# VeeraKarthick609/ImageCaptioner

Hardware: NVIDIA B200
Metric: kd_train_samples_per_sec (higher is better)
Workload: dtype bf16

## Files before the change

### imagecaptioner_b200/_ops.py

```python
from __future__ import annotations

import ctypes
import os
from typing import List, Optional, Sequence

import torch

_HERE = os.path.dirname(os.path.abspath(__file__))
LIB_PATH = os.environ.get("B2C_LIB") or os.path.join(_HERE, "lib", "libb2c.so")

B2C_MAX_LAYERS = 4
B2C_F32, B2C_BF16 = 0, 1
B2C_WS_TRAIN, B2C_WS_DECODE, B2C_WS_ATTN, B2C_WS_REFINE, B2C_WS_PROJ = 0, 1, 2, 3, 4
ABI_VERSION = 5
B2C_BWD_DEFER_JOIN = 1

c_f32p = ctypes.c_void_p


class B2CShape(ctypes.Structure):
    _fields_ = [(n, ctypes.c_int32) for n in ("B", "T", "S", "E", "H", "L", "V")]


_PARAM_FIELDS = (
    [("embedding", c_f32p), ("attn_w", c_f32p), ("attn_b", c_f32p), ("comb_w", c_f32p), ("comb_b", c_f32p)]
    + [(n, c_f32p * B2C_MAX_LAYERS) for n in ("w_ih", "w_hh", "b_ih", "b_hh")]
    + [("out0_w", c_f32p), ("out0_b", c_f32p), ("out3_w", c_f32p), ("out3_b", c_f32p)]
)


# ... 148 lines not shown
    return st


def _master(params: Sequence[torch.Tensor]) -> List[torch.Tensor]:
    out = []
    for p in params:
        q = p.detach()
        if q.dtype != torch.float32 or not q.is_contiguous():
            q = q.float().contiguous()
        out.append(q)
    return out


class CallOptions:

    def __init__(self, grad_dest=None, defer_join=False, after_backward=None, seed_dev=None, background_ctas=0):
        self.grad_dest, self.defer_join, self.after_backward, self.seed_dev = grad_dest, defer_join, after_backward, seed_dev
        self.background_ctas = background_ctas
        self.join_pending = False


_NO_OPTIONS = CallOptions()


def _options(opts) -> CallOptions:
    return opts if opts is not None else _NO_OPTIONS


def _dropout(p, seed, opts) -> B2CDropout:
    sd = opts.seed_dev
    return B2CDropout(float(p), int(seed), sd.data_ptr() if (sd is not None and float(p) > 0) else None)

# ... 120 lines not shown
        ctx.mark_non_differentiable(attw)
        return logits, hid, attw

    @staticmethod
    def backward(ctx, dlogits, dhid, _dattw):
        lib = load_library()
        shape, code, drop, L, ws, f, cap, master, hid, attw, feats_dtype, pdtypes, opts = ctx.b2c
        cdt = f.dtype
        if dlogits is None:
            dlogits = torch.zeros(shape.T, shape.B, shape.V, dtype=cdt, device=f.device)
        dlogits = dlogits.to(cdt).contiguous()
        if dhid is not None:
            dhid = dhid.to(cdt).contiguous()
        grads, all_direct = _grad_buffers(ctx.b2c_params, master, opts)
        defer = opts.defer_join and all_direct and all(dt == torch.float32 for dt in pdtypes)
        dfeats = torch.empty(shape.B, shape.S, shape.E, dtype=torch.float32, device=f.device)
        prm = _fill_struct(B2CParams(), master, L)
        grd = _fill_struct(B2CGrads(), grads, L)
        _check(lib.b2c_decoder_backward(ctypes.byref(shape), ctypes.byref(prm), f.data_ptr(), cap.data_ptr(), hid.data_ptr(), attw.data_ptr(),
                                        dlogits.data_ptr(), _ptr(dhid), ctypes.byref(grd), dfeats.data_ptr(), ws.data_ptr(), ws.numel(),
                                        code, ctypes.byref(drop), B2C_BWD_DEFER_JOIN if defer else 0, _stream()),
               "b2c_decoder_backward")
        if defer:
            opts.join_pending = True
        if opts.after_backward is not None:
            opts.after_backward()
        grads = [g if g.dtype == dt else g.to(dt) for g, dt in zip(grads, pdtypes)]
        dfe = dfeats if feats_dtype == torch.float32 else dfeats.to(feats_dtype)
        return (dfe, None, None, None, None, None, None, None, None, *grads)


def greedy_decode(feats: torch.Tensor, params: Sequence[torch.Tensor], L: int, max_len: int, start_id: int, end_id: int,
                  compute_dtype: torch.dtype = torch.float32):
    lib = load_library()
    _require_cuda(feats, "image_features")
    B, S, E = feats.shape
# ... 339 lines not shown
```

### imagecaptioner_b200/csrc/api.cu

```cuda
#include <stdlib.h>
#include "gemm.cuh"
#include "loss_kernels.cuh"
#include "decoder_kernels.cuh"
#include "recurrent.cuh"
#include "recur_cluster.cuh"
#include "refine_kernels.cuh"
#include "mha_mma.cuh"
#include "optim_kernels.cuh"

using namespace b2c;

namespace {

constexpr int MAXL = B2C_MAX_LAYERS;
constexpr int COLSUM_RS = 160;

int check_device() {
  static int cached = 1;
  if (cached <= 0) return cached;
  int dev = 0;
  B2C_CUDA(cudaGetDevice(&dev));
  int major = 0;
  B2C_CUDA(cudaDeviceGetAttribute(&major, cudaDevAttrComputeCapabilityMajor, dev));
  if (major != 10) { cached = B2C_EARCH; return set_err(B2C_EARCH, "b2c kernels are built for sm_100a only; device has compute capability major %d", major); }
// ... 25 lines not shown
template <typename T> struct Weights {
  T *Wf, *Wh, *Wce, *Wcc, *W1, *W2, *Wih0, *We; T* Wcat[MAXL]; float* bcat[MAXL]; float* bx;
  T* Wuh;
  void carve(Carver& c, const B2CShape& s) {
    Wf = c.take<T>((size_t)s.E * s.E); Wh = c.take<T>((size_t)s.E * s.H);
    Wce = c.take<T>((size_t)s.E * s.E); Wcc = c.take<T>((size_t)s.E * s.E);
    W1 = c.take<T>((size_t)s.E * s.H); W2 = c.take<T>((size_t)s.V * s.E);
    Wih0 = c.take<T>((size_t)4 * s.H * s.E); We = c.take<T>((size_t)4 * s.H * s.E); bx = c.take<float>((size_t)4 * s.H);
    for (int k = 0; k < s.L; ++k) { Wcat[k] = c.take<T>((size_t)4 * s.H * (in_dim(s, k) + s.H)); bcat[k] = c.take<float>((size_t)4 * s.H); }
    Wuh = c.take<T>((size_t)(s.E + 4 * s.H) * s.H);
  }
};

template <typename T, typename TC>
int gemm(cudaStream_t st, int M, int N, int K, const T* A, long lda, int a_mn, const T* B, long ldb, int b_mn,
         TC* C, long ldc, float beta = 0.f, const float* bias = nullptr, int relu = 0, float alpha = 1.f, int row_unperm_h = 0);

template <typename T>
int pack_params(const B2CShape& s, const B2CParams& p, const Weights<T>& w, cudaStream_t st) {
  B2C_CHECK_ARG(p.embedding && p.attn_w && p.attn_b && p.comb_w && p.comb_b && p.out0_w && p.out0_b && p.out3_w && p.out3_b, "NULL parameter pointer");
  PackTable tab; tab.n = 0;
  auto add = [&](const float* src, void* dst, int rows, int cols, long lds, long ldd, int perm_h = 0, const float* src2 = nullptr, int as_float = 0) {
    PackSeg& g = tab.seg[tab.n++]; g.src = src; g.dst = dst; g.src2 = src2; g.rows = rows; g.cols = cols; g.lds = lds; g.ldd = ldd; g.as_float = as_float; g.perm_h = perm_h;
  };
  const int E = s.E, H = s.H;
  add(p.attn_w, w.Wh, E, H, H + E, H);
  add(p.attn_w + H, w.Wf, E, E, H + E, E);
  add(p.comb_w, w.Wce, E, E, 2 * E, E);
  add(p.comb_w + E, w.Wcc, E, E, 2 * E, E);
  add(p.out0_w, w.W1, E, H, H, H);
  add(p.out3_w, w.W2, s.V, E, E, E);
// ... 96 lines not shown
  void carve(void* base, const B2CShape& s) {
    Carver c{reinterpret_cast<unsigned char*>(base), 0};
    const size_t B = s.B, S = s.S, E = s.E, H = s.H;
    w.carve(c, s);
    P = c.take<float>(B * S * E); emb = c.take<T>(B * E); u = c.take<float>(B * E); G0 = c.take<T>(B * 4 * H); o1 = c.take<T>(B * E);
    for (int k = 0; k < s.L; ++k) { xh[k] = c.take<T>(2 * B * (in_dim(s, k) + H)); this->c[k] = c.take<float>(B * H); }
    logits = c.take<float>(B * (size_t)s.V); cur = c.take<int64_t>(B); done = c.take<int32_t>(B);
    amax_v = c.take<float>(B * (size_t)cdiv(s.V, 32)); amax_i = c.take<int>(B * (size_t)cdiv(s.V, 32));
    bytes = align_up(c.off, 256);
  }
};


template <typename T, typename TC>
int gemm(cudaStream_t st, int M, int N, int K, const T* A, long lda, int a_mn, const T* B, long ldb, int b_mn,
         TC* C, long ldc, float beta, const float* bias, int relu, float alpha, int row_unperm_h) {
  GemmArgs g{M, N, K, alpha, beta, A, lda, a_mn, B, ldb, b_mn, C, ldc, bias, relu};
  g.row_unperm_h = row_unperm_h;
  return Gemm<T, TC>::run(g, st);
}
template <typename T>
int gemm_lstm(cudaStream_t st, int M, int H, int K, const T* A, long lda, const T* Wcat, long ldb, const LstmEpi& le) {
  GemmArgs g{M, 4 * H, K, 1.f, 0.f, A, lda, 0, Wcat, ldb, 0, nullptr, 4 * H, nullptr, 0};
  g.lstm = &le;
  return Gemm<T, float>::run(g, st);
}

inline int ew_grid(long n) { long g = (n + 255) / 256; if (g > 148 * 8) g = 148 * 8; if (g < 1) g = 1; return (int)g; }

template <typename T>
int colsum(cudaStream_t st, const T* A, long rows, int cols, long ld, float* partial, float* out, float* out2 = nullptr, int unperm_h = 0) {
  if (ld == cols && cols % 8 == 0 && ((uintptr_t)A & 15) == 0 && rows >= 256) {
    const int gx = cdiv(cols, 256);
// ... 294 lines not shown
  return 0;
}



inline int bg_ctas() { static int v = -1; if (v < 0) { const char* e = getenv("B2C_BG_CTAS"); v = e ? atoi(e) : 10; } return v; }
inline bool attn_post_occ3() { static int v = -1; if (v < 0) { const char* e = getenv("B2C_POST_OCC3"); v = (e && e[0] == '0') ? 0 : 1; } return v != 0; }
inline int wgrad_chunks() { static int v = -1; if (v < 0) { const char* e = getenv("B2C_WGRAD_CHUNKS"); v = e ? atoi(e) : 0; } return v; }

template <typename T>
int decoder_backward_impl(const B2CShape& s, const B2CParams& p, const T* feats, const int64_t* cap, const T* hid_top,
                          const float* attw, const T* dlogits, const T* dhid, const B2CGrads& g, float* dfeats,
                          void* ws, size_t ws_bytes, const B2CDropout& dr, cudaStream_t st, int flags) {
  TrainWs<T> W; W.carve(ws, s);
  B2C_CHECK_ARG(ws_bytes >= W.bytes, "workspace too small: %zu < %zu", ws_bytes, W.bytes);
  B2C_CHECK_ARG(g.embedding && g.attn_w && g.attn_b && g.comb_w && g.comb_b && g.out0_w && g.out0_b && g.out3_w && g.out3_b && dfeats, "NULL gradient pointer");
  const int B = s.B, Tn = s.T, S = s.S, E = s.E, H = s.H, L = s.L, V = s.V;
  const long TB = (long)Tn * B;
  const float inv_keep = dr.p > 0.f ? 1.0f / (1.0f - dr.p) : 1.0f;
  SubStreams* hs = nullptr;
  B2C_TRY(get_substreams(&hs));
  cudaStream_t side = hs->s[MAX_SUB - 1];
  for (int k = 0; k < L; ++k) B2C_CHECK_ARG(g.w_ih[k] && g.w_hh[k] && g.b_ih[k] && g.b_hh[k], "NULL LSTM gradient pointer (layer %d)", k);
  B2C_CUDA(cudaEventRecord(hs->ev[3], st));
  B2C_CUDA(cudaStreamWaitEvent(side, hs->ev[3], 0));
  B2C_CUDA(cudaMemsetAsync(W.dxh0, 0, (size_t)TB * (E + H) * sizeof(float), side));
  for (int k = 1; k < L; ++k) B2C_CUDA(cudaMemsetAsync(W.dxh[k], 0, (size_t)TB * 2 * H * sizeof(float), side));
  B2C_CUDA(cudaEventRecord(hs->ev[3], side));
  B2C_TRY((gemm<T, T>(st, (int)TB, E, V, dlogits, V, 0, W.w.W2, E, 1, W.do1, E)));
  relu_bwd_inplace_kernel<T><<<ew_grid(TB * E), 256, 0, st>>>(W.do1, W.o1, TB * E, inv_keep);
  B2C_LAUNCH_CHECK("relu_bwd_inplace_kernel");
  B2C_CUDA(cudaEventRecord(hs->fork, st));
  B2C_CUDA(cudaStreamWaitEvent(side, hs->fork, 0));
  {
    GemmCapScope bg(bg_ctas());
    B2C_TRY((gemm<T, float>(side, V, E, (int)TB, dlogits, V, 1, W.o1, E, 1, g.out3_w, E)));
    B2C_TRY(colsum<T>(side, dlogits, TB, V, V, W.partial_side, g.out3_b));
    B2C_TRY((gemm<T, float>(side, E, H, (int)TB, W.do1, E, 1, hid_top, H, 1, g.out0_w, H)));
    B2C_TRY(colsum<T>(side, W.do1, TB, E, E, W.partial_side, g.out0_b));
  }
  B2C_CUDA(cudaEventRecord(hs->join[MAX_SUB - 1], side));
  B2C_TRY((gemm<T, float>(st, (int)TB, H, E, W.do1, E, 0, W.w.W1, H, 1, W.dHext, H)));
  B2C_CUDA(cudaStreamWaitEvent(st, hs->ev[3], 0));
  SubPlan sp;
  B2C_TRY(fork_subs(sp, B, st));
  auto weight_grads = [&](cudaStream_t s2, long r0, long r1, float beta) -> int {
    const int K = (int)(r1 - r0);
    for (int k = 1; k < L; ++k) {
      const int in = in_dim(s, k), ld = in + H;
      B2C_TRY((gemm<T, float>(s2, 4 * H, in, K, W.dgates[k] + r0 * 4 * H, 4 * H, 1, W.xh[k] + r0 * ld, ld, 1, g.w_ih[k], in, beta, nullptr, 0, 1.f, H)));
      B2C_TRY((gemm<T, float>(s2, 4 * H, H, K, W.dgates[k] + r0 * 4 * H, 4 * H, 1, W.xh[k] + r0 * ld + in, ld, 1, g.w_hh[k], H, beta, nullptr, 0, 1.f, H)));
    }
    B2C_TRY((gemm<T, float>(s2, 4 * H, E, K, W.dgates[0] + r0 * 4 * H, 4 * H, 1, W.xh[0] + r0 * (E + H), E + H, 1, W.dWx32, E, beta)));
    B2C_TRY((gemm<T, float>(s2, 4 * H, E, K, W.dgates[0] + r0 * 4 * H, 4 * H, 1, W.emb + r0 * E, E, 1, W.dWe32, E, beta)));
    B2C_TRY((gemm<T, float>(s2, 4 * H, H, K, W.dgates[0] + r0 * 4 * H, 4 * H, 1, W.xh[0] + r0 * (E + H) + E, E + H, 1, g.w_hh[0], H, beta, nullptr, 0, 1.f, H)));
    return 0;
  };
  const int n_chunks = (sp.ns == 1 && bg_ctas() > 0) ? wgrad_chunks() : 0;
  const int chunk_steps = n_chunks > 0 ? cdiv(Tn, n_chunks) : 0;
  long wg_done_from = TB;
  bool wg_any = false;
  pdl_full_dependency_next();
  for (int t = Tn - 1; t >= 0; --t) {
    const bool last = (t == Tn - 1);
    for (int i = 0; i < sp.ns; ++i) {
      cudaStream_t ss = sp.st[i];
      const long b0 = sp.b0[i];
      const int Bh = sp.bn[i];
      const long row = (long)t * B + b0;
      for (int k = L - 1; k >= 0; --k) {
// ... 11 lines not shown
      }
      const float* dctx_t = W.dxh0 + row * (E + H);
      T* du_t = W.du + row * E;
      B2C_TRY(attn_bwd<T>(ss, Bh, S, E, W.P + b0 * S * E, feats + b0 * S * E, W.u + row * E, attw + row * S, dctx_t, (long)(E + H), W.ds + row * S, du_t));
      if (t > 0) B2C_TRY((gemm<T, T>(ss, Bh, H, E, du_t, E, 0, W.w.Wh, H, 1, W.dq + b0 * H, H)));
    }
    if (chunk_steps > 0 && t > 0 && (Tn - t) % chunk_steps == 0 && t >= chunk_steps) {
      B2C_CUDA(cudaEventRecord(hs->ev[0], st));
      B2C_CUDA(cudaStreamWaitEvent(side, hs->ev[0], 0));
      GemmCapScope bg(bg_ctas());
      B2C_TRY(weight_grads(side, (long)t * B, wg_done_from, wg_any ? 1.f : 0.f));
      wg_done_from = (long)t * B; wg_any = true;
    }
  }
  B2C_TRY(join_subs(sp));
  B2C_CUDA(cudaEventRecord(hs->ev[1], st));
  B2C_CUDA(cudaStreamWaitEvent(side, hs->ev[1], 0));
  B2C_TRY(weight_grads(side, 0, wg_done_from, wg_any ? 1.f : 0.f));
  for (int k = 0; k < L; ++k) B2C_TRY(colsum<T>(side, W.dgates[k], TB, 4 * H, 4 * H, W.partial_side, g.b_ih[k], g.b_hh[k], H));
  {
    cast_f32_kernel<T><<<ew_grid((long)4 * H * E / 8), 256, 0, side>>>(W.dWx32, W.dWxT, (long)4 * H * E);
    B2C_LAUNCH_CHECK("cast_f32_kernel");
    cast_f32_kernel<T><<<ew_grid((long)4 * H * E / 8), 256, 0, side>>>(W.dWe32, W.dWeT, (long)4 * H * E);
    B2C_LAUNCH_CHECK("cast_f32_kernel");
    B2C_TRY((gemm<T, float>(side, 4 * H, E, E, W.dWxT, E, 0, W.w.Wcc, E, 0, g.w_ih[0], E, 0.f, nullptr, 0, 1.f, H)));
    B2C_TRY((gemm<T, float>(side, 4 * H, E, E, W.dWeT, E, 0, W.w.Wce, E, 0, g.w_ih[0], E, 1.f, nullptr, 0, 1.f, H)));
    rank1_add_kernel<<<ew_grid((long)4 * H * E), 256, 0, side>>>(g.w_ih[0], g.b_ih[0], p.comb_b, (long)4 * H, E);
    B2C_LAUNCH_CHECK("rank1_add_kernel");
    B2C_TRY((gemm<T, float>(side, E, E, 4 * H, W.w.Wih0, E, 1, W.dWeT, E, 1, g.comb_w, 2 * E)));
    B2C_TRY((gemm<T, float>(side, E, E, 4 * H, W.w.Wih0, E, 1, W.dWxT, E, 1, g.comb_w + E, 2 * E)));
    B2C_CUDA(cudaMemsetAsync(g.comb_b, 0, (size_t)E * sizeof(float), side));
    bias_fold_bwd_kernel<<<dim3(cdiv(E, 32), 32), 256, 0, side>>>(p.w_ih[0], g.b_ih[0], 4 * H, E, g.comb_b);
    B2C_LAUNCH_CHECK("bias_fold_bwd_kernel");
    B2C_TRY((gemm<T, float>(side, (int)TB, E, 4 * H, W.dgates[0], 4 * H, 0, W.w.We, E, 1, W.demb, E)));
    B2C_CUDA(cudaMemsetAsync(g.embedding, 0, (size_t)V * E * sizeof(float), side));
    embedding_scatter_add_kernel<<<ew_grid(TB * E), 256, 0, side>>>(W.demb, cap, TB, E, V, g.embedding);
    B2C_LAUNCH_CHECK("embedding_scatter_add_kernel");
  }
  const int inL = in_dim(s, L - 1), ldL = inL + H;
  B2C_TRY((gemm<T, float>(side, E, H, (int)TB, W.du, E, 1, W.xh[L - 1] + inL, ldL, 1, g.attn_w, H + E)));
  if (Tn <= 24) {
    const int splits = 1, per = cdiv(S, splits), TP = (Tn + 3) & ~3;
    const size_t psmem = (size_t)2 * per * TP * 4;
    if (Tn <= 20 && attn_post_occ3()) {
      B2C_TRY(set_smem(attn_post_reg_kernel<T, 20>, psmem));
      attn_post_reg_kernel<T, 20><<<dim3(B, splits), ATT_THREADS, psmem, st>>>(W.P, W.u, W.dxh0, (long)(E + H), attw, W.ds, Tn, B, S, E, W.dP, dfeats);
    } else {
      B2C_TRY(set_smem(attn_post_reg_kernel<T, 24>, psmem));
      attn_post_reg_kernel<T, 24><<<dim3(B, splits), ATT_THREADS, psmem, st>>>(W.P, W.u, W.dxh0, (long)(E + H), attw, W.ds, Tn, B, S, E, W.dP, dfeats);
    }
    B2C_LAUNCH_CHECK("attn_post_reg_kernel");
  } else {
    const size_t smem = (size_t)Tn * (2 * E + 2 * S) * 4;
    B2C_TRY(set_smem(attn_post_kernel<T>, smem));
    attn_post_kernel<T><<<B, ATT_THREADS, smem, st>>>(W.P, W.u, W.dxh0, (long)(E + H), attw, W.ds, Tn, B, S, E, W.dP, dfeats);
    B2C_LAUNCH_CHECK("attn_post_kernel");
  }
  B2C_CUDA(cudaEventRecord(hs->ev[2], st));
  B2C_TRY((gemm<T, float>(st, B * S, E, E, W.dP, E, 0, W.w.Wf, E, 1, dfeats, E, 1.f)));
  B2C_CUDA(cudaStreamWaitEvent(side, hs->ev[2], 0));
  B2C_TRY((gemm<T, float>(side, E, E, B * S, W.dP, E, 1, feats, E, 1, g.attn_w + H, H + E)));
  B2C_TRY(colsum<T>(side, W.dP, (long)B * S, E, E, W.partial_side, g.attn_b));
  B2C_CUDA(cudaEventRecord(hs->join[MAX_SUB - 1], side));
  if (flags & B2C_BWD_DEFER_JOIN) return 0;
  B2C_CUDA(cudaStreamWaitEvent(st, hs->join[MAX_SUB - 1], 0));
  return 0;
}


inline bool fuse_argmax_off() { static const bool off = getenv("B2C_DECODE_LOGITS") != nullptr; return off; }

template <typename T>
int greedy_decode_impl(const B2CShape& s, const B2CParams& p, const T* feats, int64_t start_id, int64_t end_id,
                       int64_t* tokens, int32_t* lengths, void* ws, size_t ws_bytes, cudaStream_t st) {
  DecodeWs<T> W; W.carve(ws, s);
  B2C_CHECK_ARG(ws_bytes >= W.bytes, "workspace too small: %zu < %zu", ws_bytes, W.bytes);
  const int B = s.B, Tn = s.T, S = s.S, E = s.E, H = s.H, L = s.L, V = s.V;
// ... 710 lines not shown
```

### imagecaptioner_b200/csrc/gemm.cuh

```cuda
#pragma once
#include "common.cuh"

namespace b2c {

struct LstmEpi {
  int enabled, H;
  const void* addend;
  const float* bias;
  const float* c_prev; float* c_out;
  void* gates_out;
  void* h_rec; long ld_rec; void* h_next; long ld_next; void* h_top; long ld_top;
  float drop_p; unsigned long long seed; unsigned int site; long row_base;
  const unsigned long long* seed_dev;
  const float* addend32; long ld_addend32;
};

constexpr int EVAL_PART_FLOATS = 8;
struct EvalEpi { const float* teacher; const int64_t* targets; float* parts; float inv_temp; int nparts; int cols_per_part; };

struct ArgmaxEpi { float* pmax; int* pidx; int nparts; int cols_per_part; };
inline LstmEpi pack_argmax(const ArgmaxEpi& a) {
  LstmEpi le{};
  le.enabled = 2; le.H = a.nparts; le.c_out = a.pmax; le.gates_out = a.pidx; le.ld_rec = a.cols_per_part;
  return le;
// ... 515 lines not shown
          }
#pragma unroll
          for (int j = 0; j < 32; ++j) if (colb + j < N && v[j] > best) { best = v[j]; bidx = colb + j; }
        }
      }
      if (grow < M) {
        const int part = (n0 + half * C_PER * CH) / (C_PER * CH);
        if (part < nparts) { pmax[(long)grow * nparts + part] = best; pidx[(long)grow * nparts + part] = bidx; }
      }
      tc_fence_before();
      __syncwarp();
      if (lane == 0) mbar_arrive(&tempty_bar[as]);
      continue;
    }
    if constexpr (EPI == 0 || EPI == 4) {
    if (EPI == 4 || ((split ? sizeof(TC) == 4 : beta == 0.f) && vec_ok && m0 + TC_BM <= M && n0 + BN <= N && (((uintptr_t)bias) & 15) == 0)) {
#pragma unroll 1
      for (int ci = half * C_PER; ci < (half + 1) * C_PER && ci < NCHUNK; ++ci) {
        const int c0 = ci * CH;
#pragma unroll
        for (int h = 0; h < CH / 32; ++h) {
          float v[32];
          tmem_ld32(tacc + (uint32_t)(c0 + h * 32), v);
          if (add_bias) {
            const float4* b4 = reinterpret_cast<const float4*>(bias + n0 + c0 + h * 32);
#pragma unroll
            for (int j = 0; j < 8; ++j) {
              const float4 bb = __ldg(b4 + j);
              v[4 * j] = fmaf(alpha, v[4 * j], bb.x); v[4 * j + 1] = fmaf(alpha, v[4 * j + 1], bb.y);
              v[4 * j + 2] = fmaf(alpha, v[4 * j + 2], bb.z); v[4 * j + 3] = fmaf(alpha, v[4 * j + 3], bb.w);
            }
// ... 11 lines not shown
            for (int j = 0; j < 32; j += 8)
              *reinterpret_cast<uint4*>(dst + j * 2) = make_uint4(pack_bf16(v[j], v[j + 1]), pack_bf16(v[j + 2], v[j + 3]), pack_bf16(v[j + 4], v[j + 5]), pack_bf16(v[j + 6], v[j + 7]));
          } else {
#pragma unroll
            for (int j = 0; j < 32; j += 4)
              *reinterpret_cast<uint4*>(dst + j * 4) = make_uint4(__float_as_uint(v[j]), __float_as_uint(v[j + 1]), __float_as_uint(v[j + 2]), __float_as_uint(v[j + 3]));
          }
        }
        __syncwarp();
#pragma unroll
        for (int it = 0; it < 8; ++it) {
          const int r = it * 4 + (lane >> 3), grow = m0 + q * 32 + r;
          const long orow = row_unperm_h ? (long)(grow & 3) * row_unperm_h + (grow >> 2) : (long)grow;
          TC* cp = C + orow * ldc + n0 + c0 + (lane & 7) * PER;
          const uint4 acc = *reinterpret_cast<const uint4*>(my + r * TC_EPI_PITCH + (lane & 7) * 16);
          if (split) {
            asm volatile("red.global.add.v4.f32 [%0], {%1, %2, %3, %4};" :: "l"(cp), "f"(__uint_as_float(acc.x)), "f"(__uint_as_float(acc.y)),
                         "f"(__uint_as_float(acc.z)), "f"(__uint_as_float(acc.w)) : "memory");
          } else {
            *reinterpret_cast<uint4*>(cp) = acc;
          }
        }
        __syncwarp();
      }
      tc_fence_before();
      __syncwarp();
      if (lane == 0) mbar_arrive(&tempty_bar[as]);
      continue;
    }
    if constexpr (EPI == 0) {
#pragma unroll 1
// ... 108 lines not shown
  if (r != CUDA_SUCCESS) return set_err(B2C_ECUDA, "cuTensorMapEncodeTiled failed (%d): ptr=%p inner=%ld outer=%ld ld=%ld box=%d", (int)r, ptr, inner, outer, ld, box_outer);
  return 0;
}

struct GemmArgs {
  int M, N, K;
  float alpha, beta;
  const void* A; long lda; int a_mn;
  const void* B; long ldb; int b_mn;
  void* C; long ldc;
  const float* bias; int relu;
  int row_unperm_h = 0;
  const LstmEpi* lstm = nullptr;
  ArgmaxEpi* amax = nullptr;
  EvalEpi* eval = nullptr;
};

inline bool tc_eligible(const GemmArgs& g) {
  return ((uintptr_t)g.A % 16 == 0) && ((uintptr_t)g.B % 16 == 0) && (g.lda % 8 == 0) && (g.ldb % 8 == 0);
}

struct TcPlan { int bn, splits, kb_per_split; };
inline TcPlan plan_tc(const GemmArgs& g, int elem_c, int sms) {
  const int num_kb = cdiv(g.K, TC_BK);
  const bool can_split = (elem_c == 4) && !g.relu && (g.beta == 0.f || g.beta == 1.f) && (g.lstm == nullptr) && (g.amax == nullptr) && (g.eval == nullptr);
  TcPlan best{64, 1, num_kb}; double best_cost = 1e30;
  const int cand[3] = {256, 128, 64};
  for (int ci = 0; ci < 3; ++ci) {
    const int bn = cand[ci];
    if (bn > 64 && g.N <= bn / 2) continue;
// ... 23 lines not shown
  int saved;
  explicit GemmCapScope(int cap) : saved(gemm_cta_cap()) { gemm_cta_cap() = cap; }
  ~GemmCapScope() { gemm_cta_cap() = saved; }
};
inline int gemm_sms() { const int n = sm_count(), c = gemm_cta_cap(); return (c > 0 && c < n) ? c : n; }

template <int BN, bool A_MN, bool B_MN, typename TC>
int launch_tc(const GemmArgs& g, const TcPlan& plan, cudaStream_t st) {
  CUtensorMap ta, tb;
  if (!A_MN) B2C_TRY(make_tmap_bf16(&ta, g.A, g.K, g.M, g.lda, TC_BM)); else B2C_TRY(make_tmap_bf16(&ta, g.A, g.M, g.K, g.lda, 64));
  if (!B_MN) B2C_TRY(make_tmap_bf16(&tb, g.B, g.K, g.N, g.ldb, BN)); else B2C_TRY(make_tmap_bf16(&tb, g.B, g.N, g.K, g.ldb, 64));
  constexpr bool CAN_LSTM = !A_MN && !B_MN && sizeof(TC) == 4;
  void (*kern)(const CUtensorMap, const CUtensorMap, int, int, int, float, float, TC*, long, const float*, int, int, int, int, int, int, const LstmEpi) =
      gemm_tc_kernel<BN, A_MN, B_MN, TC, 0>;
  int flavour = g.lstm ? ((g.lstm->drop_p > 0.f && g.lstm->h_next) ? 1 : 5) : (g.amax ? 2 : (g.eval ? 3 : 0));
  if (flavour == 0 && fast_only_enabled() && g.M % TC_BM == 0 && g.N % BN == 0 && (plan.splits > 1 ? sizeof(TC) == 4 : g.beta == 0.f) &&
      ((uintptr_t)g.C) % 16 == 0 && (g.ldc * (long)sizeof(TC)) % 16 == 0 && (((uintptr_t)g.bias) & 15) == 0) {
    flavour = 4;
    kern = gemm_tc_kernel<BN, A_MN, B_MN, TC, 4>;
  }
  if (flavour != 0 && flavour != 4) {
    if constexpr (CAN_LSTM) {
      kern = flavour == 1 ? gemm_tc_kernel<BN, A_MN, B_MN, TC, 1> : (flavour == 5 ? gemm_tc_kernel<BN, A_MN, B_MN, TC, 5> :
             (flavour == 2 ? gemm_tc_kernel<BN, A_MN, B_MN, TC, 2> : gemm_tc_kernel<BN, A_MN, B_MN, TC, 3>));
    } else return set_err(B2C_EINVAL, "the fused LSTM / argmax / validation epilogues need K-major operands and the fp32 instantiation");
  }
  static bool attr_set[6] = {false, false, false, false, false, false};
  if (!attr_set[flavour]) {
    B2C_CUDA(cudaFuncSetAttribute(kern, cudaFuncAttributeMaxDynamicSharedMemorySize, (int)TcCfg<BN>::SMEM_BYTES));
    attr_set[flavour] = true;
  }
  const int kb_per_split = plan.kb_per_split, splits = plan.splits;
  if (splits > 1 && g.beta == 0.f)
    B2C_CUDA(cudaMemset2DAsync(g.C, (size_t)g.ldc * sizeof(TC), 0, (size_t)g.N * sizeof(TC), (size_t)g.M, st));
  const int tiles_m = cdiv(g.M, TC_BM), tiles_n = cdiv(g.N, BN);
  const long total = (long)tiles_m * tiles_n * splits;
  const int grid = (int)(total < gemm_sms() ? total : gemm_sms());
  LstmEpi epi = g.lstm ? *g.lstm : LstmEpi{};
  if (g.amax) {
    B2C_CHECK_ARG(!g.lstm && splits == 1 && g.amax->pmax && g.amax->pidx, "argmax epilogue: no K split, no LSTM epilogue, partial buffers required");
    constexpr int CHc = 128 / (int)sizeof(TC), CPER = (BN / CHc + 1) / 2;
    g.amax->cols_per_part = CPER * CHc;
    g.amax->nparts = cdiv(g.N, g.amax->cols_per_part);
    epi = pack_argmax(*g.amax);
  }
  if (g.eval) {
    B2C_CHECK_ARG(!g.lstm && !g.amax && splits == 1 && g.eval->teacher && g.eval->targets && g.eval->parts, "validation epilogue: no K split, no other epilogue, buffers required");
    constexpr int CHc = 128 / (int)sizeof(TC), CPER = (BN / CHc + 1) / 2;
// ... 48 lines not shown
```

### imagecaptioner_b200/graph.py

```python
from __future__ import annotations

import os
from typing import Dict, Optional

import torch

from . import _ops
from .ddp import FlatGradAllReducer


class GraphedKDStep:
    INPUT_KEYS = ("encoder_features", "captions_input", "targets", "teacher_logits", "teacher_features", "teacher_hiddens")

    def __init__(self, model, projector, loss_module, optimizer, reducer: Optional[FlatGradAllReducer], example: Dict[str, torch.Tensor],
                 max_grad_norm: float = 1.0, autocast_dtype: Optional[torch.dtype] = torch.bfloat16, use_graph: bool = True,
                 warmup_steps: int = 3, direct_grads: bool = True):
        self.model, self.projector, self.loss_module = model, projector, loss_module
        self._native_opt = hasattr(optimizer, "flat_param") and hasattr(optimizer, "reducer")
        if self._native_opt:
            if reducer is None:
                reducer = optimizer.reducer
            if reducer is not optimizer.reducer:
                raise ValueError("a FlatAdamW optimizer brings its own gradient buffer: pass reducer=None or optimizer.reducer")
        self.optimizer, self.reducer = optimizer, reducer
# ... 5 lines not shown
        self.static = {k: example[k].clone() for k in self.INPUT_KEYS if example.get(k) is not None}
        self.static["encoder_features"].requires_grad_(True)
        self.out5 = None
        self.graph = None
        self.graph_opt = None
        self.world = reducer.world_size
        self._side = torch.cuda.Stream()
        self._aux = torch.cuda.Stream()
        self._aux_used = False
        self._overlap = False
        self._capturing = False
        self.high_priority_chain = os.environ.get("B2C_CHAIN_PRIORITY", "1") != "0"
        self.defer_weight_grad_join = os.environ.get("B2C_DEFER_JOIN", "1") != "0"
        self.background_ctas = int(os.environ.get("B2C_BG_CTAS", "10"))
        self.direct_grads = direct_grads
        loss_module.assume_unit_grad = True
        dev = self.static["targets"].device
        self.step_counter = torch.zeros(1, dtype=torch.int64, device=dev)
        self._opts = _ops.CallOptions(grad_dest=reducer.grad_views() if direct_grads else None, seed_dev=self.step_counter)
        self._fake_dp = self.world == 1 and os.environ.get("B2C_FAKE_DP", "0") == "1"
        self._multi = self.world > 1 or self._fake_dp
        self.nval = torch.zeros(1, dtype=torch.int32, device=self.static["targets"].device) if self._multi else None
        self._nval_single = torch.zeros(1, dtype=torch.int32, device=self.static["targets"].device) if not self._multi else None
        self.overlap_comm = use_graph and self._multi and os.environ.get("B2C_OVERLAP_COMM", "1") != "0"
        self._early = self._early_segment() if self.overlap_comm else None
        if self.overlap_comm:
            self._comm = torch.cuda.Stream()
            self._ev_count = torch.cuda.Event(external=True)
            self._ev_dec = torch.cuda.Event(external=True)
        if use_graph:
# ... 20 lines not shown
            self._all_reduce(self.nval)
            self.loss_module.n_valid_global = self.nval

    def _modules(self):
        mods = [self.model.decoder, self.projector]
        if getattr(self.model, "use_attention_refinement", False):
            mods.append(self.model.attention_refinement)
        return mods

    def _attach_options(self):
        o = self._opts
        early = self._capturing and self.overlap_comm and self._early is not None
        o.defer_join = self.defer_weight_grad_join and self.direct_grads and (not self._multi or early)
        o.after_backward = self._after_decoder_backward if early else None
        o.background_ctas = self.background_ctas if self._overlap else 0
        for m in self._modules():
            m.b2c_options = o

    def _after_decoder_backward(self):
        main = torch.cuda.current_stream()
        if self._opts.join_pending:
            self._opts.join_pending = False
            self._aux.wait_stream(main)
            with torch.cuda.stream(self._aux):
                _ops.join_side_work()
                self._ev_dec.record()
            self._aux_used = True
        else:
            self._ev_dec.record()

# ... 14 lines not shown
        if feats.grad is not None:
            feats.grad = None
        self._attach_options()
        if self._dropout_active():
            _ops.bump_counter(self.step_counter)
        ctx = torch.autocast("cuda", dtype=self.autocast_dtype) if self.autocast_dtype is not None else torch.autocast("cuda", enabled=False)
        if self._overlap:
            main = torch.cuda.current_stream()
            self._side.wait_stream(main)
            if self._nval_single is not None:
                with torch.cuda.stream(self._side):
                    _ops.count_valid(inp["targets"], self.loss_module.vocab_size or 2 ** 31 - 1, out=self._nval_single)
                self.loss_module.n_valid_global = self._nval_single
            with torch.cuda.stream(self._side), ctx:
                tproj = self.projector(inp["teacher_features"])
            with ctx:
                outputs, enc, hids, _ = self.model(feats, inp["captions_input"])
            main.wait_stream(self._side)
        else:
            with ctx:
                outputs, enc, hids, _ = self.model(feats, inp["captions_input"])
                tproj = self.projector(inp["teacher_features"])
        if self._capturing and self.overlap_comm:
            torch.cuda.current_stream().wait_event(self._ev_count)
        loss, out5 = self.loss_module.forward_device(
            {"logits": outputs, "encoder_features": enc, "hidden_states": hids},
            {"logits": inp["teacher_logits"], "encoder_features": tproj, "hidden_states": inp.get("teacher_hiddens")},
            inp["targets"])
        if self.direct_grads:
            self.reducer.detach_grads()
# ... 117 lines not shown
```

### include/b2c.h

```cpp
#ifndef B2C_H_
#define B2C_H_

#include <stddef.h>
#include <stdint.h>

#ifdef __cplusplus
extern "C" {
#endif

#define B2C_ABI_VERSION 5
#define B2C_MAX_LAYERS 4

enum { B2C_OK = 0, B2C_EINVAL = -1, B2C_EARCH = -2, B2C_ECUDA = -3, B2C_ENOMEM = -4 };
enum { B2C_F32 = 0, B2C_BF16 = 1 };
enum { B2C_WS_TRAIN = 0, B2C_WS_DECODE = 1, B2C_WS_ATTN = 2, B2C_WS_REFINE = 3, B2C_WS_PROJ = 4 };

typedef struct B2CShape { int32_t B, T, S, E, H, L, V; } B2CShape;

typedef struct B2CParams {
  const float* embedding;
  const float* attn_w;  const float* attn_b;
  const float* comb_w;  const float* comb_b;
  const float* w_ih[B2C_MAX_LAYERS]; const float* w_hh[B2C_MAX_LAYERS];
  const float* b_ih[B2C_MAX_LAYERS]; const float* b_hh[B2C_MAX_LAYERS];
// ... 32 lines not shown
int b2c_decoder_prepare(const B2CShape* shape, const B2CParams* params, const int64_t* captions, void* workspace, size_t ws_bytes,
                        int dtype, void* stream);
int b2c_decoder_forward_prepared(const B2CShape* shape, const B2CParams* params, const void* feats, const int64_t* captions,
                        void* logits, void* hidden_top, float* attn_w, void* workspace, size_t ws_bytes,
                        int dtype, const B2CDropout* dropout, void* stream);

int b2c_decoder_set_initial_state(const B2CShape* shape, const float* h0, const float* c0, void* workspace, size_t ws_bytes,
                                  int dtype, void* stream);

int b2c_decoder_backward(const B2CShape* shape, const B2CParams* params, const void* feats, const int64_t* captions,
                         const void* hidden_top, const float* attn_w, const void* dlogits, const void* dhidden_top,
                         const B2CGrads* grads, float* dfeats, void* workspace, size_t ws_bytes,
                         int dtype, const B2CDropout* dropout, int flags, void* stream);

#define B2C_BWD_DEFER_JOIN 1
int b2c_join_side_work(void* stream);

int b2c_set_gemm_cta_limit(int32_t max_ctas);

int b2c_greedy_decode(const B2CShape* shape, const B2CParams* params, const void* feats, int64_t start_id, int64_t end_id,
                      int64_t* tokens, int32_t* lengths, void* workspace, size_t ws_bytes, int dtype, void* stream);

int b2c_attention_step(const B2CShape* shape, const float* attn_w, const float* attn_b, const void* hidden, const void* feats,
                       void* context, float* weights, void* workspace, size_t ws_bytes, int dtype, void* stream);

typedef struct B2CRefineParams {
  const float *in_w, *in_b, *out_w, *out_b, *ffn0_w, *ffn0_b, *ffn3_w, *ffn3_b, *n1_w, *n1_b, *n2_w, *n2_b;
} B2CRefineParams;
typedef struct B2CRefineGrads {
  float *in_w, *in_b, *out_w, *out_b, *ffn0_w, *ffn0_b, *ffn3_w, *ffn3_b, *n1_w, *n1_b, *n2_w, *n2_b;
// ... 71 lines not shown
```

Measured before the change: 208,400.

## Pre-zero gradient buffer on side stream and accumulate weight grads atomically

The flat gradient buffer is now zeroed on a side stream during the teacher projector, overlapping the forward pass. With that flag set, the backward GEMMs skip their per-GEMM memsets and write through red.global.add, and the embedding and attention weight-grad work moves to a second side stream. This removes memset launches and serialization from the backward critical path. The cost is that correctness now depends on the buffer really being zero, and atomic reductions may be slower than plain stores for non-split GEMMs.

```diff
diff --git a/imagecaptioner_b200/_ops.py b/imagecaptioner_b200/_ops.py
--- a/imagecaptioner_b200/_ops.py
+++ b/imagecaptioner_b200/_ops.py
@@ -14,6 +14,7 @@
 B2C_WS_TRAIN, B2C_WS_DECODE, B2C_WS_ATTN, B2C_WS_REFINE, B2C_WS_PROJ = 0, 1, 2, 3, 4
 ABI_VERSION = 5
 B2C_BWD_DEFER_JOIN = 1
+B2C_BWD_GRADS_ZEROED = 2
 
 c_f32p = ctypes.c_void_p
 
@@ -192,8 +193,9 @@
 
 class CallOptions:
 
-    def __init__(self, grad_dest=None, defer_join=False, after_backward=None, seed_dev=None, background_ctas=0):
+    def __init__(self, grad_dest=None, defer_join=False, after_backward=None, seed_dev=None, background_ctas=0, grads_zeroed=False):
         self.grad_dest, self.defer_join, self.after_backward, self.seed_dev = grad_dest, defer_join, after_backward, seed_dev
+        self.grads_zeroed = grads_zeroed
         self.background_ctas = background_ctas
         self.join_pending = False
 
@@ -344,12 +346,13 @@
             dhid = dhid.to(cdt).contiguous()
         grads, all_direct = _grad_buffers(ctx.b2c_params, master, opts)
         defer = opts.defer_join and all_direct and all(dt == torch.float32 for dt in pdtypes)
+        flags = (B2C_BWD_DEFER_JOIN if defer else 0) | (B2C_BWD_GRADS_ZEROED if opts.grads_zeroed and all_direct else 0)
         dfeats = torch.empty(shape.B, shape.S, shape.E, dtype=torch.float32, device=f.device)
         prm = _fill_struct(B2CParams(), master, L)
         grd = _fill_struct(B2CGrads(), grads, L)
         _check(lib.b2c_decoder_backward(ctypes.byref(shape), ctypes.byref(prm), f.data_ptr(), cap.data_ptr(), hid.data_ptr(), attw.data_ptr(),
                                         dlogits.data_ptr(), _ptr(dhid), ctypes.byref(grd), dfeats.data_ptr(), ws.data_ptr(), ws.numel(),
-                                        code, ctypes.byref(drop), B2C_BWD_DEFER_JOIN if defer else 0, _stream()),
+                                        code, ctypes.byref(drop), flags, _stream()),
                "b2c_decoder_backward")
         if defer:
             opts.join_pending = True
diff --git a/imagecaptioner_b200/csrc/api.cu b/imagecaptioner_b200/csrc/api.cu
--- a/imagecaptioner_b200/csrc/api.cu
+++ b/imagecaptioner_b200/csrc/api.cu
@@ -63,7 +63,8 @@
 
 template <typename T, typename TC>
 int gemm(cudaStream_t st, int M, int N, int K, const T* A, long lda, int a_mn, const T* B, long ldb, int b_mn,
-         TC* C, long ldc, float beta = 0.f, const float* bias = nullptr, int relu = 0, float alpha = 1.f, int row_unperm_h = 0);
+         TC* C, long ldc, float beta = 0.f, const float* bias = nullptr, int relu = 0, float alpha = 1.f, int row_unperm_h = 0,
+         bool c_zeroed = false);
 
 template <typename T>
 int pack_params(const B2CShape& s, const B2CParams& p, const Weights<T>& w, cudaStream_t st) {
@@ -190,9 +191,10 @@
 
 template <typename T, typename TC>
 int gemm(cudaStream_t st, int M, int N, int K, const T* A, long lda, int a_mn, const T* B, long ldb, int b_mn,
-         TC* C, long ldc, float beta, const float* bias, int relu, float alpha, int row_unperm_h) {
+         TC* C, long ldc, float beta, const float* bias, int relu, float alpha, int row_unperm_h, bool c_zeroed) {
   GemmArgs g{M, N, K, alpha, beta, A, lda, a_mn, B, ldb, b_mn, C, ldc, bias, relu};
   g.row_unperm_h = row_unperm_h;
+  g.c_zeroed = c_zeroed;
   return Gemm<T, TC>::run(g, st);
 }
 template <typename T>
@@ -517,6 +519,7 @@
                           void* ws, size_t ws_bytes, const B2CDropout& dr, cudaStream_t st, int flags) {
   TrainWs<T> W; W.carve(ws, s);
   B2C_CHECK_ARG(ws_bytes >= W.bytes, "workspace too small: %zu < %zu", ws_bytes, W.bytes);
+  const bool zg = (flags & B2C_BWD_GRADS_ZEROED) != 0;
   B2C_CHECK_ARG(g.embedding && g.attn_w && g.attn_b && g.comb_w && g.comb_b && g.out0_w && g.out0_b && g.out3_w && g.out3_b && dfeats, "NULL gradient pointer");
   const int B = s.B, Tn = s.T, S = s.S, E = s.E, H = s.H, L = s.L, V = s.V;
   const long TB = (long)Tn * B;
@@ -529,6 +532,10 @@
   B2C_CUDA(cudaStreamWaitEvent(side, hs->ev[3], 0));
   B2C_CUDA(cudaMemsetAsync(W.dxh0, 0, (size_t)TB * (E + H) * sizeof(float), side));
   for (int k = 1; k < L; ++k) B2C_CUDA(cudaMemsetAsync(W.dxh[k], 0, (size_t)TB * 2 * H * sizeof(float), side));
+  if (zg) {
+    B2C_CUDA(cudaMemsetAsync(W.dWx32, 0, (size_t)4 * H * E * sizeof(float), side));
+    B2C_CUDA(cudaMemsetAsync(W.dWe32, 0, (size_t)4 * H * E * sizeof(float), side));
+  }
   B2C_CUDA(cudaEventRecord(hs->ev[3], side));
   B2C_TRY((gemm<T, T>(st, (int)TB, E, V, dlogits, V, 0, W.w.W2, E, 1, W.do1, E)));
   relu_bwd_inplace_kernel<T><<<ew_grid(TB * E), 256, 0, st>>>(W.do1, W.o1, TB * E, inv_keep);
@@ -537,9 +544,9 @@
   B2C_CUDA(cudaStreamWaitEvent(side, hs->fork, 0));
   {
     GemmCapScope bg(bg_ctas());
-    B2C_TRY((gemm<T, float>(side, V, E, (int)TB, dlogits, V, 1, W.o1, E, 1, g.out3_w, E)));
+    B2C_TRY((gemm<T, float>(side, V, E, (int)TB, dlogits, V, 1, W.o1, E, 1, g.out3_w, E, 0.f, nullptr, 0, 1.f, 0, zg)));
     B2C_TRY(colsum<T>(side, dlogits, TB, V, V, W.partial_side, g.out3_b));
-    B2C_TRY((gemm<T, float>(side, E, H, (int)TB, W.do1, E, 1, hid_top, H, 1, g.out0_w, H)));
+    B2C_TRY((gemm<T, float>(side, E, H, (int)TB, W.do1, E, 1, hid_top, H, 1, g.out0_w, H, 0.f, nullptr, 0, 1.f, 0, zg)));
     B2C_TRY(colsum<T>(side, W.do1, TB, E, E, W.partial_side, g.out0_b));
   }
   B2C_CUDA(cudaEventRecord(hs->join[MAX_SUB - 1], side));
@@ -551,12 +558,12 @@
     const int K = (int)(r1 - r0);
     for (int k = 1; k < L; ++k) {
       const int in = in_dim(s, k), ld = in + H;
-      B2C_TRY((gemm<T, float>(s2, 4 * H, in, K, W.dgates[k] + r0 * 4 * H, 4 * H, 1, W.xh[k] + r0 * ld, ld, 1, g.w_ih[k], in, beta, nullptr, 0, 1.f, H)));
-      B2C_TRY((gemm<T, float>(s2, 4 * H, H, K, W.dgates[k] + r0 * 4 * H, 4 * H, 1, W.xh[k] + r0 * ld + in, ld, 1, g.w_hh[k], H, beta, nullptr, 0, 1.f, H)));
+      B2C_TRY((gemm<T, float>(s2, 4 * H, in, K, W.dgates[k] + r0 * 4 * H, 4 * H, 1, W.xh[k] + r0 * ld, ld, 1, g.w_ih[k], in, beta, nullptr, 0, 1.f, H, zg)));
+      B2C_TRY((gemm<T, float>(s2, 4 * H, H, K, W.dgates[k] + r0 * 4 * H, 4 * H, 1, W.xh[k] + r0 * ld + in, ld, 1, g.w_hh[k], H, beta, nullptr, 0, 1.f, H, zg)));
     }
-    B2C_TRY((gemm<T, float>(s2, 4 * H, E, K, W.dgates[0] + r0 * 4 * H, 4 * H, 1, W.xh[0] + r0 * (E + H), E + H, 1, W.dWx32, E, beta)));
-    B2C_TRY((gemm<T, float>(s2, 4 * H, E, K, W.dgates[0] + r0 * 4 * H, 4 * H, 1, W.emb + r0 * E, E, 1, W.dWe32, E, beta)));
-    B2C_TRY((gemm<T, float>(s2, 4 * H, H, K, W.dgates[0] + r0 * 4 * H, 4 * H, 1, W.xh[0] + r0 * (E + H) + E, E + H, 1, g.w_hh[0], H, beta, nullptr, 0, 1.f, H)));
+    B2C_TRY((gemm<T, float>(s2, 4 * H, E, K, W.dgates[0] + r0 * 4 * H, 4 * H, 1, W.xh[0] + r0 * (E + H), E + H, 1, W.dWx32, E, beta, nullptr, 0, 1.f, 0, zg)));
+    B2C_TRY((gemm<T, float>(s2, 4 * H, E, K, W.dgates[0] + r0 * 4 * H, 4 * H, 1, W.emb + r0 * E, E, 1, W.dWe32, E, beta, nullptr, 0, 1.f, 0, zg)));
+    B2C_TRY((gemm<T, float>(s2, 4 * H, H, K, W.dgates[0] + r0 * 4 * H, 4 * H, 1, W.xh[0] + r0 * (E + H) + E, E + H, 1, g.w_hh[0], H, beta, nullptr, 0, 1.f, H, zg)));
     return 0;
   };
   const int n_chunks = (sp.ns == 1 && bg_ctas() > 0) ? wgrad_chunks() : 0;
@@ -598,8 +605,17 @@
     }
   }
   B2C_TRY(join_subs(sp));
+  cudaStream_t side2 = hs->s[MAX_SUB - 2];
   B2C_CUDA(cudaEventRecord(hs->ev[1], st));
   B2C_CUDA(cudaStreamWaitEvent(side, hs->ev[1], 0));
+  B2C_CUDA(cudaStreamWaitEvent(side2, hs->ev[1], 0));
+  B2C_TRY((gemm<T, float>(side2, (int)TB, E, 4 * H, W.dgates[0], 4 * H, 0, W.w.We, E, 1, W.demb, E)));
+  if (!zg) B2C_CUDA(cudaMemsetAsync(g.embedding, 0, (size_t)V * E * sizeof(float), side2));
+  embedding_scatter_add_kernel<<<ew_grid(TB * E), 256, 0, side2>>>(W.demb, cap, TB, E, V, g.embedding);
+  B2C_LAUNCH_CHECK("embedding_scatter_add_kernel");
+  const int inL = in_dim(s, L - 1), ldL = inL + H;
+  B2C_TRY((gemm<T, float>(side2, E, H, (int)TB, W.du, E, 1, W.xh[L - 1] + inL, ldL, 1, g.attn_w, H + E, 0.f, nullptr, 0, 1.f, 0, zg)));
+  B2C_CUDA(cudaEventRecord(hs->join[MAX_SUB - 2], side2));
   B2C_TRY(weight_grads(side, 0, wg_done_from, wg_any ? 1.f : 0.f));
   for (int k = 0; k < L; ++k) B2C_TRY(colsum<T>(side, W.dgates[k], TB, 4 * H, 4 * H, W.partial_side, g.b_ih[k], g.b_hh[k], H));
   {
@@ -611,18 +627,12 @@
     B2C_TRY((gemm<T, float>(side, 4 * H, E, E, W.dWeT, E, 0, W.w.Wce, E, 0, g.w_ih[0], E, 1.f, nullptr, 0, 1.f, H)));
     rank1_add_kernel<<<ew_grid((long)4 * H * E), 256, 0, side>>>(g.w_ih[0], g.b_ih[0], p.comb_b, (long)4 * H, E);
     B2C_LAUNCH_CHECK("rank1_add_kernel");
-    B2C_TRY((gemm<T, float>(side, E, E, 4 * H, W.w.Wih0, E, 1, W.dWeT, E, 1, g.comb_w, 2 * E)));
-    B2C_TRY((gemm<T, float>(side, E, E, 4 * H, W.w.Wih0, E, 1, W.dWxT, E, 1, g.comb_w + E, 2 * E)));
-    B2C_CUDA(cudaMemsetAsync(g.comb_b, 0, (size_t)E * sizeof(float), side));
+    B2C_TRY((gemm<T, float>(side, E, E, 4 * H, W.w.Wih0, E, 1, W.dWeT, E, 1, g.comb_w, 2 * E, 0.f, nullptr, 0, 1.f, 0, zg)));
+    B2C_TRY((gemm<T, float>(side, E, E, 4 * H, W.w.Wih0, E, 1, W.dWxT, E, 1, g.comb_w + E, 2 * E, 0.f, nullptr, 0, 1.f, 0, zg)));
+    if (!zg) B2C_CUDA(cudaMemsetAsync(g.comb_b, 0, (size_t)E * sizeof(float), side));
     bias_fold_bwd_kernel<<<dim3(cdiv(E, 32), 32), 256, 0, side>>>(p.w_ih[0], g.b_ih[0], 4 * H, E, g.comb_b);
     B2C_LAUNCH_CHECK("bias_fold_bwd_kernel");
-    B2C_TRY((gemm<T, float>(side, (int)TB, E, 4 * H, W.dgates[0], 4 * H, 0, W.w.We, E, 1, W.demb, E)));
-    B2C_CUDA(cudaMemsetAsync(g.embedding, 0, (size_t)V * E * sizeof(float), side));
-    embedding_scatter_add_kernel<<<ew_grid(TB * E), 256, 0, side>>>(W.demb, cap, TB, E, V, g.embedding);
-    B2C_LAUNCH_CHECK("embedding_scatter_add_kernel");
-  }
-  const int inL = in_dim(s, L - 1), ldL = inL + H;
-  B2C_TRY((gemm<T, float>(side, E, H, (int)TB, W.du, E, 1, W.xh[L - 1] + inL, ldL, 1, g.attn_w, H + E)));
+  }
   if (Tn <= 24) {
     const int splits = 1, per = cdiv(S, splits), TP = (Tn + 3) & ~3;
     const size_t psmem = (size_t)2 * per * TP * 4;
@@ -643,8 +653,9 @@
   B2C_CUDA(cudaEventRecord(hs->ev[2], st));
   B2C_TRY((gemm<T, float>(st, B * S, E, E, W.dP, E, 0, W.w.Wf, E, 1, dfeats, E, 1.f)));
   B2C_CUDA(cudaStreamWaitEvent(side, hs->ev[2], 0));
-  B2C_TRY((gemm<T, float>(side, E, E, B * S, W.dP, E, 1, feats, E, 1, g.attn_w + H, H + E)));
+  B2C_TRY((gemm<T, float>(side, E, E, B * S, W.dP, E, 1, feats, E, 1, g.attn_w + H, H + E, 0.f, nullptr, 0, 1.f, 0, zg)));
   B2C_TRY(colsum<T>(side, W.dP, (long)B * S, E, E, W.partial_side, g.attn_b));
+  B2C_CUDA(cudaStreamWaitEvent(side, hs->join[MAX_SUB - 2], 0));
   B2C_CUDA(cudaEventRecord(hs->join[MAX_SUB - 1], side));
   if (flags & B2C_BWD_DEFER_JOIN) return 0;
   B2C_CUDA(cudaStreamWaitEvent(st, hs->join[MAX_SUB - 1], 0));
diff --git a/imagecaptioner_b200/csrc/gemm.cuh b/imagecaptioner_b200/csrc/gemm.cuh
--- a/imagecaptioner_b200/csrc/gemm.cuh
+++ b/imagecaptioner_b200/csrc/gemm.cuh
@@ -553,7 +553,7 @@
       continue;
     }
     if constexpr (EPI == 0 || EPI == 4) {
-    if (EPI == 4 || ((split ? sizeof(TC) == 4 : beta == 0.f) && vec_ok && m0 + TC_BM <= M && n0 + BN <= N && (((uintptr_t)bias) & 15) == 0)) {
+    if (EPI == 4 || (((split || beta == 1.f) ? sizeof(TC) == 4 : beta == 0.f) && vec_ok && m0 + TC_BM <= M && n0 + BN <= N && (((uintptr_t)bias) & 15) == 0)) {
 #pragma unroll 1
       for (int ci = half * C_PER; ci < (half + 1) * C_PER && ci < NCHUNK; ++ci) {
         const int c0 = ci * CH;
@@ -595,7 +595,7 @@
           const long orow = row_unperm_h ? (long)(grow & 3) * row_unperm_h + (grow >> 2) : (long)grow;
           TC* cp = C + orow * ldc + n0 + c0 + (lane & 7) * PER;
           const uint4 acc = *reinterpret_cast<const uint4*>(my + r * TC_EPI_PITCH + (lane & 7) * 16);
-          if (split) {
+          if (split || beta != 0.f) {
             asm volatile("red.global.add.v4.f32 [%0], {%1, %2, %3, %4};" :: "l"(cp), "f"(__uint_as_float(acc.x)), "f"(__uint_as_float(acc.y)),
                          "f"(__uint_as_float(acc.z)), "f"(__uint_as_float(acc.w)) : "memory");
           } else {
@@ -734,6 +734,7 @@
   const LstmEpi* lstm = nullptr;
   ArgmaxEpi* amax = nullptr;
   EvalEpi* eval = nullptr;
+  bool c_zeroed = false;
 };
 
 inline bool tc_eligible(const GemmArgs& g) {
@@ -787,7 +788,7 @@
   void (*kern)(const CUtensorMap, const CUtensorMap, int, int, int, float, float, TC*, long, const float*, int, int, int, int, int, int, const LstmEpi) =
       gemm_tc_kernel<BN, A_MN, B_MN, TC, 0>;
   int flavour = g.lstm ? ((g.lstm->drop_p > 0.f && g.lstm->h_next) ? 1 : 5) : (g.amax ? 2 : (g.eval ? 3 : 0));
-  if (flavour == 0 && fast_only_enabled() && g.M % TC_BM == 0 && g.N % BN == 0 && (plan.splits > 1 ? sizeof(TC) == 4 : g.beta == 0.f) &&
+  if (flavour == 0 && fast_only_enabled() && g.M % TC_BM == 0 && g.N % BN == 0 && ((plan.splits > 1 || g.beta == 1.f) ? sizeof(TC) == 4 : g.beta == 0.f) &&
       ((uintptr_t)g.C) % 16 == 0 && (g.ldc * (long)sizeof(TC)) % 16 == 0 && (((uintptr_t)g.bias) & 15) == 0) {
     flavour = 4;
     kern = gemm_tc_kernel<BN, A_MN, B_MN, TC, 4>;
@@ -804,7 +805,7 @@
     attr_set[flavour] = true;
   }
   const int kb_per_split = plan.kb_per_split, splits = plan.splits;
-  if (splits > 1 && g.beta == 0.f)
+  if (splits > 1 && g.beta == 0.f && !g.c_zeroed)
     B2C_CUDA(cudaMemset2DAsync(g.C, (size_t)g.ldc * sizeof(TC), 0, (size_t)g.N * sizeof(TC), (size_t)g.M, st));
   const int tiles_m = cdiv(g.M, TC_BM), tiles_n = cdiv(g.N, BN);
   const long total = (long)tiles_m * tiles_n * splits;
diff --git a/imagecaptioner_b200/graph.py b/imagecaptioner_b200/graph.py
--- a/imagecaptioner_b200/graph.py
+++ b/imagecaptioner_b200/graph.py
@@ -43,6 +43,7 @@
         self.defer_weight_grad_join = os.environ.get("B2C_DEFER_JOIN", "1") != "0"
         self.background_ctas = int(os.environ.get("B2C_BG_CTAS", "10"))
         self.direct_grads = direct_grads
+        self.prezero_grads = os.environ.get("B2C_PREZERO_GRADS", "1") != "0"
         loss_module.assume_unit_grad = True
         dev = self.static["targets"].device
         self.step_counter = torch.zeros(1, dtype=torch.int64, device=dev)
@@ -93,6 +94,7 @@
         o.defer_join = self.defer_weight_grad_join and self.direct_grads and (not self._multi or early)
         o.after_backward = self._after_decoder_backward if early else None
         o.background_ctas = self.background_ctas if self._overlap else 0
+        o.grads_zeroed = self.prezero_grads and self.direct_grads and self._overlap
         for m in self._modules():
             m.b2c_options = o
 
@@ -137,6 +139,8 @@
                 self.loss_module.n_valid_global = self._nval_single
             with torch.cuda.stream(self._side), ctx:
                 tproj = self.projector(inp["teacher_features"])
+                if self._opts.grads_zeroed:
+                    self.reducer.flat.zero_()
             with ctx:
                 outputs, enc, hids, _ = self.model(feats, inp["captions_input"])
             main.wait_stream(self._side)
diff --git a/include/b2c.h b/include/b2c.h
--- a/include/b2c.h
+++ b/include/b2c.h
@@ -70,6 +70,7 @@
                          int dtype, const B2CDropout* dropout, int flags, void* stream);
 
 #define B2C_BWD_DEFER_JOIN 1
+#define B2C_BWD_GRADS_ZEROED 2
 int b2c_join_side_work(void* stream);
 
 int b2c_set_gemm_cta_limit(int32_t max_ctas);
```

Result: faster. 214,500, median of 6 (+2.9%).
